# PimLb/POMDP_PBVI_Exploration

Hardware: AMD Instinct MI355X
Metric: alpha-vector backups/sec (higher is better)
Workload: dtype f32

## Files before the change

pomdp_pbvi_exploration_amd/csrc/backup_kernels.h:

```cpp
#pragma once
#include "pbvi_common.h"

namespace pbvi {

template <typename T>
struct ModelView {
    int S, S_pad, A, O, R;
    const int32_t* rs;
    const T* rto;
    const T* er;
    const uint8_t* sup;
};

__host__ __device__ __forceinline__ int64_t push_row_index(int o, int a, int b, int A, int B) {
#ifdef PBVI_PUSH_ORDER_OAB
    return ((int64_t)o * A + a) * B + b;
#else
    return ((int64_t)o * B + b) * A + a;
#endif
}

template <typename T>
struct SlabView {
    const T* slabs;
// ... 51 lines not shown
hipError_t launch_dead(const T* bel, int ldb, int B, ModelView<T> mv,
                       const unsigned long long* nzBw ,
                       int k_tiles, uint8_t* dead, int32_t* btl ,
                       int32_t* btc , int* dead_count ,
                       hipStream_t st, const uint8_t* rowflags = nullptr ,
                       const int32_t* perm = nullptr );

template <typename T>
hipError_t launch_push_project(const T* bel, int ldb, int B, ModelView<T> mv, const int32_t* in_ptr,
                               const int32_t* in_src, double gamma, const T* amax, T* bp, int ldp, double* mag,
                               hipStream_t st, uint8_t* nzP = nullptr );
template <typename T>
hipError_t launch_rdot(const T* bel, int ldb, int B, ModelView<T> mv, const int32_t* btl, const int32_t* btc, double* rd,
                       hipStream_t st);

template <typename T>
hipError_t launch_argmax(SlabView<T> sv, int V, int G, int B, const uint8_t* dead, double tol_rel, double tol_abs,
                         const int* chain_steps ,
                         int flag_all, int32_t* best_v, double* best_score, double* err, int32_t* queue, int* qcount,
                         hipStream_t st, double tol_extra = 0.0 ,
                         int split = 0 );

template <typename T>
hipError_t launch_fold_chunk(SlabView<T> sv, int B, int G, int Vc, int V, int v0, int tail_cols, T* dst, int64_t ldd,
                             const int* chain, int* chain_max, hipStream_t st);

struct RefineWork {
    int32_t* items_v = nullptr;
    int32_t* items_slot = nullptr;
    double* scores = nullptr;
    int32_t* slot_entry = nullptr;
    int32_t* slot_n = nullptr;
    int32_t* tiles = nullptr;
    unsigned long long* emax = nullptr;
    int32_t* eidx = nullptr;
    double* ib_val = nullptr;
// ... 15 lines not shown
    int* klistW = nullptr;
    int* kcountW = nullptr;
    const int32_t* in_ptr = nullptr;
    const int32_t* in_src = nullptr;
    const float* gam = nullptr;
    int ldg = 0;
    double l1_rel = 0.0;
};

template <typename T, typename TS>
hipError_t launch_refine(bool proj, SlabView<TS> sv, int V, int G, int max_entries, const int32_t* queue,
                         const int* qcount, const T* bel, int ldb, const T* alpha, int lda, ModelView<T> mv,
                         double gamma, const int32_t* btl, const int32_t* btc ,
                         const uint8_t* nzG ,
                         int32_t* best_v, double* best_score, double* err, int* cand_total ,
                         RefineWork work, hipStream_t st);

template <typename T, typename TS>
hipError_t launch_refine_scan(bool proj, SlabView<TS> sv, int V, int G, int max_entries, const int32_t* queue,
                              const int* qcount, const T* bel, int ldb, const T* alpha, int lda, ModelView<T> mv,
                              double gamma, const int32_t* btl, const int32_t* btc, const uint8_t* nzG, int32_t* best_v,
                              double* best_score, double* err, int* cand_total, RefineWork work, int* counts_host,
                              hipStream_t st);
template <typename T>
hipError_t launch_refine_deferred(bool proj, int V, int G, const T* bel, int ldb, const T* alpha, int lda, ModelView<T> mv,
                                  double gamma, int32_t* best_v, double* best_score, double* err, RefineWork work,
                                  int h_items, int h_slots, hipStream_t st);

template <typename T>
hipError_t launch_belief_tiles(const T* bel, int ldb, int B, int S, int k_tiles, int32_t* btl, int32_t* btc,
                               hipStream_t st);

template <typename T>
hipError_t launch_tail_rows(ModelView<T> mv, T* gam , int64_t row0 , int ldg, hipStream_t st,
                            const int32_t* ctile = nullptr);
template <typename T>
hipError_t launch_action(int B, ModelView<T> mv, SlabView<T> sv, int64_t rd_col0, double tol_rel, const int* chain_steps,
                         const double* best_score, const double* err, double* rdot, double* rdot_err, int32_t* action,
// ... 46 lines not shown
```

pomdp_pbvi_exploration_amd/csrc/backup_kernels.hip:

```cpp
#include "backup_kernels.h"

#include <cstdlib>
#include <limits>

namespace pbvi {

__device__ __forceinline__ double wave_sum(double v) {
#pragma unroll
    for (int off = 32; off > 0; off >>= 1) v += __shfl_xor(v, off, 64);
    return v;
}

__device__ __forceinline__ double block_sum(double v, double* sh) {
    v = wave_sum(v);
    const int lane = threadIdx.x & 63, wid = threadIdx.x >> 6;
    __syncthreads();
    if (lane == 0) sh[wid] = v;
    __syncthreads();
    return ((sh[0] + sh[1]) + sh[2]) + sh[3];
}

struct TileList {
    const int32_t* list;
    int count;
// ... 567 lines not shown
    return hipGetLastError();
}

__device__ __forceinline__ double score_window(double tol_rel, const int* chain_steps, int split) {
    const double u24 = 5.9604644775390625e-08;
    double tr = tol_rel;
    if (chain_steps != nullptr && tol_rel < 0.0)
        tr = 8.0 * u24 * (sqrt((double)chain_steps[0] * 32.0 * (split ? 3.0 : 1.0)) + 1.0);
    if (split) tr = (tr + 3.1 * 1.52587890625e-05) * (1.0 + 4.8828125e-04);
    return tr;
}

template <typename T>
__global__ void k_argmax(SlabView<T> sv, int V, int G, int B, const uint8_t* __restrict__ dead, double tol_rel,
                         double tol_abs, double tol_extra, const int* __restrict__ chain_steps, int flag_all, int32_t* __restrict__ best_v, double* __restrict__ best_score,
                         double* __restrict__ err, int32_t* __restrict__ queue, int* __restrict__ qcount, int split) {
    const int lane = threadIdx.x & 63;
    const int64_t gw = (int64_t)blockIdx.x * 4 + (threadIdx.x >> 6);
    if (gw >= (int64_t)B * G) return;
    const int b = (int)(gw / G), g = (int)(gw % G);
    if (dead != nullptr && dead[gw]) {
        if (lane == 0) {
            best_v[gw] = 0;
            best_score[gw] = 0.0;
            err[gw] = 0.0;
        }
        return;
    }
    T m = -std::numeric_limits<T>::infinity(), m2 = -std::numeric_limits<T>::infinity();
    int idx = 0x7fffffff;
    bool vec4 = false;
// ... 81 lines not shown
        if (oi != 0x7fffffff && idx != 0x7fffffff) n2 = lo > n2 ? lo : n2;
        if (om > m || (om == m && oi < idx)) {
            m = om;
            idx = oi;
        }
        m2 = n2;
    }
    double E = 0.0;
    int push = 0;
    if (queue != nullptr) {
        const double mag = fmax(fabs((double)m), fabs(sv.magnitude(b, g, G, V)));
        const double tr = score_window(tol_rel, chain_steps, split) + (sv.push ? 2.0 * 5.9604644775390625e-08 : 0.0);
        E = (tr + tol_extra) * mag + tol_abs;
        push = (flag_all || (double)m2 >= (double)m - 2.0 * E) ? 1 : 0;
    }
    if (lane == 0) {
        best_v[gw] = idx;
        best_score[gw] = (double)m;
        err[gw] = E;
        if (push) {
            const int slot = atomicAdd(qcount, 1);
            queue[slot] = (int32_t)gw;
        }
    }
}

template <typename T>
hipError_t launch_argmax(SlabView<T> sv, int V, int G, int B, const uint8_t* dead, double tol_rel, double tol_abs,
                         const int* chain_steps, int flag_all, int32_t* best_v, double* best_score, double* err,
                         int32_t* queue, int* qcount, hipStream_t st, double tol_extra, int split) {
    const int64_t rows = (int64_t)B * G;
    if (rows <= 0) return hipSuccess;
    hipLaunchKernelGGL(k_argmax<T>, dim3((unsigned)((rows + 3) / 4)), dim3(256), 0, st, sv, V, G, B, dead, tol_rel,
                       tol_abs, tol_extra, chain_steps, flag_all, best_v, best_score, err, queue, qcount, split);
    return hipGetLastError();
}

template <typename T>
__global__ void k_fold_chunk(SlabView<T> sv, int B, int G, int Vc, int V, int v0, int tail_cols, T* __restrict__ dst,
                             int64_t ldd, const int* __restrict__ chain, int* __restrict__ chain_max) {
    if (chain != nullptr && blockIdx.x == 0 && blockIdx.y == 0 && threadIdx.x == 0) {
        const int c = chain[0];
        if (c > chain_max[0]) chain_max[0] = c;
    }
    const int64_t group_cols = (int64_t)G * Vc, n_cols = group_cols + tail_cols;
    const int64_t j0 = ((int64_t)blockIdx.x * 256 + threadIdx.x) * 4;
    if (j0 >= n_cols) return;
    bool vec4 = false;
    if constexpr (sizeof(T) == 4) vec4 = sv.nchunks != nullptr && (Vc & 3) == 0 && (sv.ldc & 3) == 0 && j0 + 3 < group_cols;
// ... 81 lines not shown
            }
#pragma unroll
            for (int j = 0; j < 4; ++j) acc[j] += w[j] * ((double)brow[s[j]] * (gamma * g[j]));
        } else {
#pragma unroll
            for (int j = 0; j < 4; ++j) {
                const bool in = s[j] < mv.S;
                acc[j] += (in ? w[j] : 0.0) * ((double)brow[s[j]] * (double)arow[in ? s[j] : 0]);
            }
        }
    }
    return wave_sum((acc[0] + acc[1]) + (acc[2] + acc[3]));
}

template <typename T, typename TS, bool PROJ, bool L1 >
__global__ void k_refine(SlabView<TS> sv, int V, int G, const int32_t* __restrict__ queue,
                         const int* __restrict__ qcount,
                         const T* __restrict__ bel, int ldb, const T* __restrict__ alpha, int lda,
                         ModelView<T> mv, double gamma, const int32_t* __restrict__ btl, const int32_t* __restrict__ btc,
                         const uint8_t* __restrict__ nzG ,
                         int32_t* __restrict__ best_v,
                         double* __restrict__ best_score, double* __restrict__ err, int* __restrict__ cand_total,
                         RefineWork work) {
    __shared__ int cand[256];
    __shared__ int wcount[4];
    __shared__ int ltile[REFINE_LIST_CAP];
    __shared__ int lbase, loverflow;
    __shared__ int sh_slot, sh_base;
    __shared__ double red[4];
    __shared__ double wbest[4];
    __shared__ int widx[4];
    if ((int)blockIdx.x >= *qcount) return;
    const int tid = threadIdx.x, lane = tid & 63, wid = tid >> 6;
    const int e = queue[blockIdx.x];
    const int b = e / G, g = e % G;
    const int a = PROJ ? g / mv.O : 0, o = PROJ ? g % mv.O : 0;
    const double m = best_score[e], E = err[e];
    const double thr = m - 2.0 * E;
    const T* brow = bel + (int64_t)b * ldb;
    const int k_tiles = mv.S_pad >> 5;
    const int32_t* src = btl ? btl + (int64_t)b * k_tiles : nullptr;
    const int n_src = btl ? btc[b] : k_tiles;
    const uint8_t* zg = (PROJ && nzG) ? nzG + (int64_t)g * k_tiles : nullptr;
    if (tid == 0) {
        lbase = 0;
        loverflow = 0;
    }
    __syncthreads();
    for (int i0 = 0; i0 < n_src; i0 += 256) {
        const int i = i0 + tid;
        int t = 0, f = 0;
        if (i < n_src) {
            t = src ? src[i] : i;
            f = zg ? (zg[t] != 0) : 1;
        }
        const unsigned long long mask = __ballot(f);
        if (lane == 0) wcount[wid] = __popcll(mask);
        __syncthreads();
        int off = lbase;
        for (int w = 0; w < wid; ++w) off += wcount[w];
        const int tot = wcount[0] + wcount[1] + wcount[2] + wcount[3];
        const bool fits = lbase + tot <= REFINE_LIST_CAP;
        if (f && fits) ltile[off + __popcll(mask & ((1ull << lane) - 1ull))] = t;
        __syncthreads();
        if (tid == 0) {
            if (fits) lbase += tot;
            else loverflow = 1;
        }
        __syncthreads();
        if (loverflow) break;
    }
    const int* L = loverflow ? src : ltile;
    const int n_tiles = loverflow ? n_src : lbase;

    double bestval = -std::numeric_limits<double>::infinity();
    int bestidx = 0x7fffffff;
    int slot = -1;
    if (tid == 0) sh_slot = -1;
    auto score_exact = [&](int ncand) {
        if (ncand <= 2) {
            const TileList tl{L, n_tiles};
            for (int c = 0; c < ncand; ++c) {
                const int vv = cand[c];
                const T* arow = alpha + (int64_t)vv * lda;
                const double part = PROJ ? proj_dot_partial(brow, arow, mv, a, o, gamma, tl)
// ... 11 lines not shown
                if (tot > bestval) {
                    bestval = tot;
                    bestidx = vv;
                }
            }
        }
    };
    bool settled = false;
    if (!loverflow) {
        constexpr int L1_CAP = 32;
        constexpr int FAST_CAP = 8;
        __shared__ int c1[L1_CAP];
        __shared__ double s1[L1_CAP];
        __shared__ double l1red[16];
        __shared__ int n1_sh, n2_sh;
        if (tid == 0) n1_sh = 0;
        __syncthreads();
        for (int v0 = 0; v0 < V; v0 += 256) {
            const int v = v0 + tid;
            int flag = 0;
            if (v < V) flag = ((double)sv.score(b, g, V, v) >= thr) ? 1 : 0;
            const unsigned long long mask = __ballot(flag);
            if (lane == 0) wcount[wid] = __popcll(mask);
            __syncthreads();
            int base = n1_sh;
            for (int w = 0; w < wid; ++w) base += wcount[w];
            const int pos = base + __popcll(mask & ((1ull << lane) - 1ull));
            if (flag && pos < L1_CAP) c1[pos] = v;
            __syncthreads();
            if (tid == 0) n1_sh += wcount[0] + wcount[1] + wcount[2] + wcount[3];
            __syncthreads();
        }
        const int n1 = n1_sh;
        constexpr bool l1 = L1 && PROJ && sizeof(T) == 4;
        if (n1 > 0 && n1 <= L1_CAP && (l1 || n1 <= FAST_CAP)) {
            if (tid == 0 && cand_total != nullptr) atomicAdd(cand_total, n1);
            const TileList tl{L, n_tiles};
            int n2 = n1;
            if constexpr (l1) {
                {
                    for (int c0 = 0; c0 < n1; c0 += 4) {
                        const float* rows[4];
#pragma unroll
                        for (int j = 0; j < 4; ++j)
                            rows[j] = work.gam + ((int64_t)g * V + c1[c0 + j < n1 ? c0 + j : c0]) * work.ldg;
                        double d[4];
// ... 138 lines not shown
                bv = wbest[w];
                bi = widx[w];
            }
        if (slot >= 0 && slot < work.w_slot_cap) {
        } else if (slot >= 0) {
            work.ib_val[slot] = bv;
            work.ib_idx[slot] = bi;
        } else if (bi != 0x7fffffff) {
            best_v[e] = bi;
            best_score[e] = bv;
            err[e] = 0.0;
        }
    }
}

template <typename T, bool PROJ>
__global__ void k_refine_split(int G, const T* __restrict__ bel, int ldb, const T* __restrict__ alpha, int lda, ModelView<T> mv,
                               double gamma, const int32_t* __restrict__ btl, const int32_t* __restrict__ btc,
                               const uint8_t* __restrict__ nzG, int32_t* __restrict__ best_v, double* __restrict__ best_score,
                               double* __restrict__ err, RefineWork work) {
    __shared__ int wcount[4];
    __shared__ int ltile[REFINE_LIST_CAP];
    __shared__ int lbase, loverflow, last;
    __shared__ double red16[16];
    const int tid = threadIdx.x, lane = tid & 63, wid = tid >> 6, part = blockIdx.y;
    const int n_q = min(work.cnt[2], work.q2_cap);
    const int k_tiles = mv.S_pad >> 5;
    for (int q = blockIdx.x; q < n_q; q += gridDim.x) {
        const int e = work.q2_entry[q], nc_all = work.q2_n[q];
        const int b = e / G, g = e % G;
// ... 197 lines not shown
    if (tid == 0) {
        for (int w = 1; w < 4; ++w)
            if (wv[w] > m || (wv[w] == m && wi[w] < idx)) {
                m = wv[w];
                idx = wi[w];
            }
        if (idx != 0x7fffffff) {
            const int e = work.slot_entry[sl];
            best_v[e] = idx;
            best_score[e] = m;
            err[e] = 0.0;
        }
    }
}

template <typename T, typename TS>
hipError_t launch_refine_scan(bool proj, SlabView<TS> sv, int V, int G, int max_entries, const int32_t* queue,
                              const int* qcount, const T* bel, int ldb, const T* alpha, int lda, ModelView<T> mv,
                              double gamma, const int32_t* btl, const int32_t* btc, const uint8_t* nzG, int32_t* best_v,
                              double* best_score, double* err, int* cand_total, RefineWork work, int* counts_host,
                              hipStream_t st) {
    if (max_entries <= 0) return hipSuccess;
    hipError_t e;
    if (work.items_v != nullptr) {
        if ((e = hipMemsetAsync(work.cnt, 0, work.zero_bytes, st)) != hipSuccess) return e;
    }
    if (proj)
    {
        if (work.gam != nullptr && sizeof(T) == 4) {
            hipLaunchKernelGGL((k_refine<T, TS, true, true>), dim3(max_entries), dim3(256), 0, st, sv, V, G, queue, qcount, bel, ldb,
                               alpha, lda, mv, gamma, btl, btc, nzG, best_v, best_score, err, cand_total, work);
            if (work.q2_entry != nullptr)
                hipLaunchKernelGGL((k_refine_split<T, true>), dim3(work.q2_cap < 256 ? work.q2_cap : 256, REFINE_SPLIT), dim3(256), 0,
                                   st, G, bel, ldb, alpha, lda, mv, gamma, btl, btc, nzG, best_v, best_score, err, work);
        } else
            hipLaunchKernelGGL((k_refine<T, TS, true, false>), dim3(max_entries), dim3(256), 0, st, sv, V, G, queue, qcount, bel, ldb,
                               alpha, lda, mv, gamma, btl, btc, nzG, best_v, best_score, err, cand_total, work);
    }
    else
        hipLaunchKernelGGL((k_refine<T, TS, false, false>), dim3(max_entries), dim3(256), 0, st, sv, V, G, queue, qcount, bel,
                           ldb, alpha, lda, mv, gamma, btl, btc, nzG, best_v, best_score, err, cand_total, work);
    if ((e = hipGetLastError()) != hipSuccess) return e;
    if (work.items_v != nullptr && counts_host != nullptr)
        if ((e = hipMemcpyAsync(counts_host, work.cnt, 2 * sizeof(int), hipMemcpyDeviceToHost, st)) != hipSuccess) return e;
    return hipSuccess;
}

template <typename T>
hipError_t launch_refine_deferred(bool proj, int V, int G, const T* bel, int ldb, const T* alpha, int lda, ModelView<T> mv,
                                  double gamma, int32_t* best_v, double* best_score, double* err, RefineWork work,
                                  int h_items, int h_slots, hipStream_t st) {
    hipError_t e;
    if (work.items_v == nullptr) return hipSuccess;
    const int n_items = h_items < work.item_cap ? h_items : work.item_cap;
    const int n_slots = h_slots < work.slot_cap ? h_slots : work.slot_cap;
    const int n_w = n_slots < work.w_slot_cap ? n_slots : work.w_slot_cap;
// ... 30 lines not shown
        else
            hipLaunchKernelGGL((k_refine_items<T, false>), dim3(blocks), dim3(256), 0, st, G, bel, ldb, alpha, lda, mv,
                               gamma, work);
        if ((e = hipGetLastError()) != hipSuccess) return e;
        hipLaunchKernelGGL(k_refine_first, dim3(1024), dim3(256), 0, st, work);
        if ((e = hipGetLastError()) != hipSuccess) return e;
    }
    if (n_slots > n_w) hipLaunchKernelGGL(k_refine_merge, dim3(64), dim3(256), 0, st, work, best_v, best_score, err);
    return hipGetLastError();
}

template <typename T, typename TS>
hipError_t launch_refine(bool proj, SlabView<TS> sv, int V, int G, int max_entries, const int32_t* queue,
                         const int* qcount, const T* bel, int ldb, const T* alpha, int lda, ModelView<T> mv,
                         double gamma, const int32_t* btl, const int32_t* btc, const uint8_t* nzG, int32_t* best_v,
                         double* best_score, double* err, int* cand_total, RefineWork work, hipStream_t st) {
    if (max_entries <= 0) return hipSuccess;
    int h_cnt[2] = {0, 0};
    hipError_t e = launch_refine_scan<T, TS>(proj, sv, V, G, max_entries, queue, qcount, bel, ldb, alpha, lda, mv, gamma, btl,
                                             btc, nzG, best_v, best_score, err, cand_total, work, h_cnt, st);
    if (e != hipSuccess || work.items_v == nullptr) return e;
    if ((e = hipStreamSynchronize(st)) != hipSuccess) return e;
    return launch_refine_deferred<T>(proj, V, G, bel, ldb, alpha, lda, mv, gamma, best_v, best_score, err, work, h_cnt[0],
                                     h_cnt[1], st);
}

template <typename T>
__global__ void k_tail_rows(ModelView<T> mv, T* __restrict__ gam, int64_t row0, int ldg, const int32_t* __restrict__ ctile) {
    const int s = blockIdx.x * 256 + threadIdx.x;
    const int j = blockIdx.y;
    if (s >= mv.S_pad) return;
    const T e = mv.er[(int64_t)(j % mv.A) * mv.S_pad + s];
    const int64_t row = row0 + j;
    const int64_t at = ctile != nullptr ? (int64_t)ctile[row >> 8] * 256 + (row & 255) : row;
    gam[at * ldg + s] = (j < mv.A) ? e : (e < T(0) ? -e : e);
// ... 646 lines not shown
    if (e != hipSuccess) return e;
    hipLaunchKernelGGL(k_walk_norm<T>, dim3(blocks), dim3(256), 0, st, unnorm, partial, blocks, mv.S, mv.S_pad, out64,
                       out_store);
    return hipGetLastError();
}

#define PBVI_INST(T)                                                                                                   \
    template hipError_t launch_support<T>(ModelView<T>, uint8_t*, hipStream_t);                                        \
    template hipError_t launch_project<T>(const T*, int, int, ModelView<T>, T, T*, int, const uint8_t*, int,           \
                                          hipStream_t, const uint8_t*, const int*, int, const int32_t*, const int32_t*); \
    template hipError_t launch_tail_rows<T>(ModelView<T>, T*, int64_t, int, hipStream_t, const int32_t*);               \
    template hipError_t launch_dead<T>(const T*, int, int, ModelView<T>, const unsigned long long*, int, uint8_t*, int32_t*, \
                                       int32_t*, int*, hipStream_t, const uint8_t*, const int32_t*);                                                   \
    template hipError_t launch_belief_tiles<T>(const T*, int, int, int, int, int32_t*, int32_t*, hipStream_t);         \
    template hipError_t launch_argmax<T>(SlabView<T>, int, int, int, const uint8_t*, double, double, const int*, int,  \
                                         int32_t*, double*, double*, int32_t*, int*, hipStream_t, double, int);        \
    template hipError_t launch_fold_chunk<T>(SlabView<T>, int, int, int, int, int, int, T*, int64_t, const int*, int*,   \
                                             hipStream_t);                                                             \
    template hipError_t launch_refine<T, T>(bool, SlabView<T>, int, int, int, const int32_t*, const int*, const T*, int, \
                                         const T*, int, ModelView<T>, double, const int32_t*, const int32_t*,          \
                                         const uint8_t*, int32_t*, double*, double*, int*, RefineWork, hipStream_t);   \
    template hipError_t launch_action<T>(int, ModelView<T>, SlabView<T>, int64_t, double, const int*, const double*,   \
                                         const double*, double*, double*, int32_t*, int32_t*, int*, hipStream_t, double, uint8_t*, \
                                         int);                                                                          \
    template hipError_t launch_refine_action<T>(const T*, int, int, const T*, int, ModelView<T>, double,               \
                                                const int32_t*, const int32_t*, const int32_t*, const int*,            \
                                                const double*, const double*, const int32_t*, const double*,           \
                                                const double*, double*, int32_t*, hipStream_t, const uint8_t*);                        \
    template hipError_t launch_assemble<T>(const T*, int, ModelView<T>, double, const int32_t*, const int32_t*,        \
                                           const int32_t*, const int*, int, T*, int, hipStream_t);                     \
    template hipError_t launch_expand_rows<T>(const T*, const int32_t*, T*, int, int, hipStream_t);                    \
    template hipError_t launch_keep<T>(const T*, int, const T*, int, int, int, const double*, const int32_t*,          \
                                       const int32_t*, uint8_t*, hipStream_t);                                         \
    template hipError_t launch_belief_update<T>(const T*, int, int, ModelView<T>, const int32_t*, const int32_t*,      \
                                                const int32_t*, const int32_t*, const int32_t*, double*, double*, T*,  \
                                                int, hipStream_t);                                                     \
// ... 2 lines not shown
    template hipError_t launch_rdot<T>(const T*, int, int, ModelView<T>, const int32_t*, const int32_t*, double*,      \
                                       hipStream_t);                                                                   \
    template hipError_t launch_walk_step<T>(const double*, ModelView<T>, const double*, const int32_t*, const int32_t*, \
                                            int, int, double*, double*, double*, T*, hipStream_t);                     \
    template hipError_t launch_walk_fused<T>(const double*, const double*, const double*, double*, T*, ModelView<T>,      \
                                             const double*, const int32_t*, const int32_t*, int, int, double*, double*,   \
                                             hipStream_t);                                                               \
    template hipError_t launch_walk_finish<T>(const double*, const double*, ModelView<T>, double*, T*, hipStream_t);     \
    template hipError_t launch_dominated<T>(const T*, int, int, int, int*, hipStream_t);
PBVI_INST(float)
PBVI_INST(double)
#define PBVI_INST_REFINE(T, TS)                                                                                        \
    template hipError_t launch_refine_scan<T, TS>(bool, SlabView<TS>, int, int, int, const int32_t*, const int*, const T*, \
                                                  int, const T*, int, ModelView<T>, double, const int32_t*, const int32_t*, \
                                                  const uint8_t*, int32_t*, double*, double*, int*, RefineWork, int*,   \
                                                  hipStream_t);
PBVI_INST_REFINE(float, float)
PBVI_INST_REFINE(double, double)
PBVI_INST_REFINE(double, float)
template hipError_t launch_refine_deferred<float>(bool, int, int, const float*, int, const float*, int, ModelView<float>, double,
                                                  int32_t*, double*, double*, RefineWork, int, int, hipStream_t);
template hipError_t launch_refine_deferred<double>(bool, int, int, const double*, int, const double*, int, ModelView<double>,
                                                   double, int32_t*, double*, double*, RefineWork, int, int, hipStream_t);
template hipError_t launch_refine<double, float>(bool, SlabView<float>, int, int, int, const int32_t*, const int*, const double*,
                                                 int, const double*, int, ModelView<double>, double, const int32_t*,
                                                 const int32_t*, const uint8_t*, int32_t*, double*, double*, int*, RefineWork,
                                                 hipStream_t);

}
```

pomdp_pbvi_exploration_amd/csrc/engine.hip:

```cpp
#include <algorithm>
#include <cmath>
#include <cstdio>
#include <cstdlib>
#include <cstring>
#include <condition_variable>
#include <mutex>
#include <new>
#include <string>
#include <thread>
#include <unistd.h>
#include <vector>

#include "backup_kernels.h"
#include "split_bf16.h"

namespace pbvi {

static thread_local std::string g_err;
static int g_poison = -1;
static bool poison_enabled() {
    if (g_poison < 0) g_poison = getenv("PBVI_POISON") != nullptr ? 1 : 0;
    return g_poison == 1;
}
void set_error(const std::string& msg) { g_err = msg; }
// ... 586 lines not shown
        const int64_t n = (V + lo - 1) / lo;
        Vc = round_up((V + n - 1) / n, 4);
    }
    out->chunk_rows = Vc;
    out->n_chunks = (V + Vc - 1) / Vc;
    out->bytes = bytes_of(Vc);
    return out->bytes <= budget ? PBVI_OK : PBVI_ENOMEM;
}

struct ScoreIO {
    int32_t* best_v;
    double* best_score;
    double* err;
    int32_t* queue;
    int* qcount;
    const uint8_t* dead;
    const double* prd;
    hipEvent_t join;
    hipStream_t side;
    hipEvent_t* ev;
    bool stats;
    double tol_extra;
    bool allow_split;
};
template <typename TS>
struct ScoreStage {
    SlabView<TS> sv;
    GemmPlan plan;
    double tol_rel;
    const int* chain;
// ... 74 lines not shown
    double tie_rel_user_ = -1.0;

    DevBuf rs_, rto_, er_, sup_;
    DevBuf alpha_, alpha_buf_, alpha_small_;
    std::vector<int32_t> prim_ids_;
    int64_t prim_off_ = 0;
    bool prim_valid_ = false, alpha_on_primary_ = false;
    uint64_t prim_layout_ver_ = 0;
    uint64_t screen_layout_seen_ = 0;
    int64_t screen_off_seen_ = 0;
    int64_t V_ = 0;
    DevBuf bel_;
    int64_t B_ = 0, B_pad_ = 0;
    DevBuf belsp_;
    uint64_t belsp_ver_ = 0;
    DevBuf gam_, slabs_, best_v_, best_score_, err_, dead_, queue_, counters_, rdot_, action_, aqueue_, out_, keep_;
    DevBuf bv2_, bs2_, err2_, queue2_, prune_cnt_;
    int tiling_mode_ = 0;
    int64_t tiling_rows_ = 0;
    DevBuf scores_, chain_max_;
    std::vector<hipEvent_t> tile_ev_;
    int tile_ev_chunks_ = 0;
    DevBuf stage_, keys_, perm_, action_res_, best_res_;
    DevBuf rep_, uniq_, inv_, slot_, out_full_;
    DevBuf store_[2], ids_;
    int64_t store_rows_[2] = {0, 0};
    DevBuf in_ptr_, in_src_, bu_act_, bu_obs_, bu_row_, bu_unnorm_, bu_mass_, bu_out_, walk64_, rto64_;
    std::vector<int32_t> h_rs_;
    DevBuf btl_, btc_, val_exact_;
    DevBuf bp_, nzP_, pmag_, prd_;
    bool btl_valid_ = false;
// ... 77 lines not shown
    bool owns_streams_ = true;
    EngineT<float>* screen_ = nullptr;
    std::vector<int32_t> h_reach_ref_;
    std::vector<double> h_rto_ref_, h_er_ref_;
    uint64_t alpha_ver_ = 1, bel_ver_ = 1;
    uint64_t screen_alpha_seen_ = 0, screen_bel_seen_ = 0;

    ~EngineT() override {
        (void)hipSetDevice(device_);
        if (screen_) {
            (void)hipStreamSynchronize(stream_);
            delete screen_;
            screen_ = nullptr;
        }
        DevBuf* all[] = {&rs_, &rto_, &er_, &sup_, &alpha_buf_, &alpha_small_, &bel_, &belsp_, &gam_, &slabs_, &best_v_, &best_score_, &err_,
                         &dead_, &queue_, &counters_, &rdot_, &action_, &aqueue_, &out_, &keep_, &bv2_, &bs2_,
                         &err2_, &queue2_, &prune_cnt_, &nzB_, &nzA_, &klist_, &kcount_, &nchunks_, &need_, &skws_, &stage_, &keys_, &perm_,
                         &action_res_, &best_res_, &rep_, &uniq_, &inv_, &slot_, &out_full_, &btl_, &btc_, &val_exact_, &store_[0], &store_[1], &ids_, &in_ptr_, &in_src_, &bu_act_, &bu_obs_,
                         &bu_unnorm_, &bu_mass_, &bu_out_, &bu_row_, &walk64_, &rto64_, &bp_, &nzP_, &pmag_, &prd_, &keys_tmp_, &keys_act_, &keys_best_, &keys_rows_, &rf_v_, &rf_slot_, &rf_sc_, &rf_entry_, &rf_n_, &rf_tiles_,
                         &snz_, &sbtl_, &sbtc_, &vmax_bk_, &rf_ibv_, &rf_ibi_, &rf_cnt_, &rf_W_, &rf_Cx_, &rf_nzW_, &rf_klW_, &rf_kcW_,
                         &dense_, &nzD_, &nzAlpha_, &prod_, &klistD_, &kcountD_, &nchunksD_, &mat_, &vlist_, &irr_, &rowflags_, &nzBw_, &scr_flag_, &ctile_, &acand_, &rf_q2_, &rf_q2p_, &rf_q2d_, &e_bv_, &e_bs_, &e_err_, &e_rdot_, &e_act_, &e_ares_, &e_bres_, &e_rep_, &e_uniq_, &e_inv_, &e_slotd_, &e_cnt_, &e_out_, &e_slot_, &scores_, &chain_max_};
        static const bool dbg = getenv("PBVI_DEBUG") != nullptr;
        auto chk = [&](hipError_t e, const char* what) {
            if (e != hipSuccess && dbg) fprintf(stderr, "[pbvi] engine teardown: %s: %s\n", what, hipGetErrorString(e));
        };
        for (auto& e : walk_ev_)
            if (e) chk(hipEventDestroy(e), "hipEventDestroy(walk)");
        for (DevBuf* b : all) b->release();
        for (auto& e : tile_ev_)
            if (e) chk(hipEventDestroy(e), "hipEventDestroy(tile)");
        if (host_stage_) chk(hipHostFree(host_stage_), "hipHostFree(stage)");
// ... 700 lines not shown
        int rc = keys_tmp_.ensure((size_t)n * sizeof(uint64_t), &bytes_);
        if (rc) return rc;
        hipLaunchKernelGGL(k_row_hash<double>, dim3((unsigned)n), dim3(256), 0, stream_, walk64_.as<double>() + S_, S_, S_,
                           keys_tmp_.as<unsigned long long>());
        HIPCHK(hipGetLastError());
        if ((rc = out_begin())) return rc;
        if ((rc = out_add(out_keys, keys_tmp_.p, (size_t)n * sizeof(uint64_t)))) return rc;
        return out_finish();
    }

    int after_oom() override {
        HIPCHK(hipSetDevice(device_));
        (void)hipStreamSynchronize(stream_);
        if (stream2_) (void)hipStreamSynchronize(stream2_);
        if (stream3_) (void)hipStreamSynchronize(stream3_);
        DevBuf* drop[] = {&alpha_buf_, &alpha_small_, &bel_, &belsp_, &gam_, &slabs_, &best_v_, &best_score_, &err_, &dead_, &queue_, &rdot_,
                          &action_, &aqueue_, &out_, &keep_, &bv2_, &bs2_, &err2_, &queue2_, &prune_cnt_, &nzA_, &klist_, &kcount_,
                          &nchunks_, &need_, &skws_, &stage_, &keys_, &perm_, &action_res_, &best_res_, &rep_, &uniq_, &inv_, &slot_,
                          &out_full_, &btl_, &btc_, &val_exact_, &store_[0], &store_[1], &ids_, &bu_act_, &bu_obs_, &bu_unnorm_,
                          &bu_mass_, &bu_out_, &bu_row_, &walk64_, &bp_, &nzP_, &pmag_, &prd_, &keys_tmp_, &keys_act_, &keys_best_,
                          &keys_rows_, &rf_v_, &rf_slot_, &rf_sc_, &rf_entry_, &rf_n_, &rf_tiles_, &snz_, &sbtl_, &sbtc_, &vmax_bk_,
                          &rf_ibv_, &rf_ibi_, &rf_cnt_, &rf_W_, &rf_Cx_, &rf_nzW_, &rf_klW_, &rf_kcW_, &nzAlpha_, &prod_, &klistD_,
                          &kcountD_, &nchunksD_, &mat_, &vlist_, &rowflags_, &ctile_, &acand_, &rf_q2_, &rf_q2p_, &rf_q2d_, &e_bv_, &e_bs_, &e_err_, &e_rdot_, &e_act_, &e_ares_, &e_bres_, &e_rep_, &e_uniq_, &e_inv_, &e_slotd_, &e_out_, &e_slot_, &scores_};
        for (DevBuf* b : drop) {
            bytes_ -= (int64_t)b->cap;
            b->release();
        }
        alpha_ = DevBuf{};
        V_ = 0;
        B_ = B_pad_ = 0;
        prim_valid_ = alpha_on_primary_ = false;
// ... 1130 lines not shown
        int split = want_split;
        if ((rc = score_gemm(gam_.as<T>(), N, nzB_.as<uint8_t>(), AO, (int)V_, &sv, nullptr, 0, nullptr, io.side, fused, &split)))
            return rc;
        out->split = split;
        out->fused = fused != nullptr;
    }
    HIPCHK(hipEventRecord(io.ev[2], stream_));
    HIPCHK(hipStreamWaitEvent(stream_, io.join, 0));
    out->plan = plan_;
    const int k_chunk = kF32 ? plan_.chunk_len * GEMM_BK : S_pad_;
    out->tol_rel = tie_window(k_chunk);
    out->chain = chain_steps();
    out->rd_col0 = (int64_t)AO * Vt;
    out->f64_pairs = f64_pairs_;
    HIPCHK(launch_argmax<T>(sv, (int)V_, AO, (int)B_, io.dead, out->tol_rel, 0.0, out->chain, 0, io.best_v, io.best_score,
                            io.err, io.queue, io.qcount, stream_, io.tol_extra, out->split));
    HIPCHK(hipEventRecord(io.ev[3], stream_));
    out->sv = sv;
    return PBVI_OK;
}

template <typename T>
int EngineT<T>::ensure_exact(DevBuf& b, size_t bytes) {
    if (bytes > b.cap && b.p != nullptr) {
        HIPCHK(hipStreamSynchronize(stream_));
        bytes_ -= (int64_t)b.cap;
        b.release();
    }
    return b.ensure(bytes, &bytes_);
}

// ... 72 lines not shown
    full.slabs = scores_.as<T>();
    full.slab_stride = 0;
    full.ldc = (int)ldd;
    full.nchunks = nullptr;
    full.tiles_m = 0;
    full.fixed = 1;
    out->plan = plan_;
    out->tol_rel = on_device ? -1.0 : tol;
    out->chain = on_device ? chain_max_.as<int>() : nullptr;
    out->rd_col0 = (int64_t)AO * Vt;
    out->extra_row0 = -1;
    out->f64_pairs = f64_pairs_;
    out->fused = false;
    out->chunks = (int)n_chunks;
    HIPCHK(launch_argmax<T>(full, (int)V_, AO, (int)B_, io.dead, out->tol_rel, 0.0, out->chain, 0, io.best_v, io.best_score,
                            io.err, io.queue, io.qcount, stream_, io.tol_extra, out->split));
    HIPCHK(hipEventRecord(io.ev[3], stream_));
    out->sv = full;
    return PBVI_OK;
}

template <typename T>
int EngineT<T>::ensure_screen() {
    if constexpr (kF32) {
        return PBVI_OK;
    } else {
        if (screen_) return PBVI_OK;
        if (h_rto_ref_.empty()) FAIL(PBVI_ERUNTIME, "screen: host tables were not kept");
        std::vector<float> rto32(h_rto_ref_.begin(), h_rto_ref_.end()), er32(h_er_ref_.begin(), h_er_ref_.end());
        auto* e = new (std::nothrow) EngineT<float>();
        if (!e) FAIL(PBVI_ENOMEM, "screen: host allocation failed");
// ... 106 lines not shown
    constexpr bool windows = sizeof(TS) == 4;
    constexpr bool screened = sizeof(TS) != sizeof(T);
    int rc;
    const int AO = A_ * O_;
    const int64_t Vt = V_ + 1;
    const int64_t N = (int64_t)AO * Vt + 2 * A_;
    const int64_t pairs = B_ * AO;
    if (N > 0x7fffffff || pairs > 0x7fffffff) FAIL(PBVI_EUNSUPPORTED, "backup_run: A*O*(V+1) or B*A*O exceeds int32");
    const ModelView<T> mv = view();
    const bool use_push = scorer.choose_push(N);
    last_formulation_ = use_push ? 2 : 1;
    if ((rc = best_v_.ensure((size_t)pairs * sizeof(int32_t), &bytes_))) return rc;
    if ((rc = best_score_.ensure((size_t)pairs * sizeof(double), &bytes_))) return rc;
    if ((rc = err_.ensure((size_t)pairs * sizeof(double), &bytes_))) return rc;
    if ((rc = queue_.ensure((size_t)pairs * sizeof(int32_t), &bytes_))) return rc;
    if ((rc = dead_.ensure((size_t)pairs, &bytes_))) return rc;
    if ((rc = rdot_.ensure((size_t)B_ * A_ * 2 * sizeof(double), &bytes_))) return rc;
    if ((rc = action_.ensure((size_t)B_ * sizeof(int32_t), &bytes_))) return rc;
    if ((rc = aqueue_.ensure((size_t)B_ * sizeof(int32_t), &bytes_))) return rc;
    if ((rc = acand_.ensure((size_t)B_ * A_, &bytes_))) return rc;
    if ((rc = out_.ensure((size_t)B_ * S_ * sizeof(T), &bytes_))) return rc;
    if ((rc = keep_.ensure((size_t)B_, &bytes_))) return rc;
    int* qcount = counters_.as<int>();
    int* aqcount = counters_.as<int>() + 1;
    if (windows && (rc = stage_reserve(256))) return rc;
    HIPCHK(hipMemsetAsync(counters_.p, 0, 8 * sizeof(int), stream_));

    HIPCHK(hipEventRecord(ev_[0], stream_));
    static const bool no_side = getenv("PBVI_NO_SIDE_STREAM") != nullptr;
    hipStream_t side = no_side ? stream_ : stream2_;
// ... 27 lines not shown
                              windows ? btc_.as<int32_t>() : nullptr, prd_.as<double>(), side));
    }
    const bool early_wanted = windows && early_rows_ != nullptr && !(flags & PBVI_BELIEF_DOMINANCE) && early_cap_ >= B_ && !no_side;
    if (early_wanted) {
        if ((rc = e_cnt_.ensure(4 * sizeof(int), &bytes_))) return rc;
        HIPCHK(hipMemsetAsync(e_cnt_.p, 0, 4 * sizeof(int), side));
    }
    HIPCHK(hipEventRecord(ev_join_, side));

    ScoreIO io;
    io.best_v = best_v_.as<int32_t>();
    io.best_score = best_score_.as<double>();
    io.err = err_.as<double>();
    io.queue = windows ? queue_.as<int32_t>() : nullptr;
    io.qcount = qcount;
    io.dead = windows ? dead_.as<uint8_t>() : nullptr;
    io.prd = use_push ? prd_.as<double>() : nullptr;
    io.join = ev_join_;
    io.side = lists;
    io.ev = ev_;
    io.stats = st != nullptr;
    io.tol_extra = screened ? 4.0 * 5.9604644775390625e-08 : 0.0;
    io.allow_split = !screened;
    if (windows && !use_push && scorer.tiling_mode_ != 0) {
        RefineWork reserve;
        if ((rc = refine_work(pairs, V_, &reserve))) return rc;
    }
    ScoreStage<TS> sc;
    if ((rc = scorer.stage_scores(gamma, use_push, io, &sc))) return rc;
    const SlabView<TS>& sv = sc.sv;
// ... 87 lines not shown
            if (!no_l1 && !use_push && !sc.fused && sc.chunks <= 1 && mode_ == PBVI_SPARSE) {
                work.gam = (const float*)gam_.p;
                work.ldg = S_pad_;
                work.l1_rel = (double)(R_ + 4) * 5.9604644775390625e-08;
            }
        }
        rf_counts_ = pinned_flag();
        if (!rf_counts_) FAIL(PBVI_ENOMEM, "backup_run: pinned flag");
        rf_counts_ += 24;
        rf_counts_[0] = rf_counts_[1] = 0;
        static const bool no_spec = getenv("PBVI_NO_SPECULATION") != nullptr;
        speculate = !no_spec && last_deferred_nothing_ && work.items_v != nullptr && !(flags & PBVI_BELIEF_DOMINANCE);
        HIPCHK((launch_refine_scan<T, TS>(true, sv, (int)V_, AO, (int)pairs, queue_.as<int32_t>(), qcount, bel_.as<T>(), S_pad_,
                                          alpha_.as<T>(), S_pad_, mv, gamma, btl_.as<int32_t>(), btc_.as<int32_t>(),
                                          nzB_.as<uint8_t>(), best_v_.as<int32_t>(), best_score_.as<double>(), err_.as<double>(),
                                          counters_.as<int>() + 4, work, rf_counts_, stream_)));
        if (!speculate && work.items_v != nullptr) {
            HIPCHK(hipStreamSynchronize(stream_));
            last_deferred_nothing_ = rf_counts_[0] == 0 && rf_counts_[1] == 0;
            HIPCHK(launch_refine_deferred<T>(true, (int)V_, AO, bel_.as<T>(), S_pad_, alpha_.as<T>(), S_pad_, mv, gamma,
                                             best_v_.as<int32_t>(), best_score_.as<double>(), err_.as<double>(), work,
                                             rf_counts_[0], rf_counts_[1], stream_));
        }
    }
    if (early_used_ && early_dma_pending_) {
        HIPCHK(hipEventSynchronize(ev_early_[0]));
        const int np = h_flag_[8];
        if (np > 0)
            HIPCHK(hipMemcpyAsync(early_rows_, e_out_.p, (size_t)np * S_ * sizeof(T), hipMemcpyDeviceToHost, stream2_));
        HIPCHK(hipEventRecord(ev_early_[1], stream2_));
        early_dma_pending_ = false;
// ... 699 lines not shown
```

Measured before the change: 654,800.

## Precompute refine candidate lists in argmax and make refine grid persistent

The argmax kernel now records, for each queued pair, up to a small fixed number of near-best candidate vectors, and the refine kernel reuses that list instead of rescanning all V scores. The refine kernel also becomes a persistent grid capped at resident occupancy that loops over queue entries, and it builds the tile list with a single-wave ballot compaction instead of block-wide atomics. The aim is to cut redundant score scans and block launch overhead in refine. The cost is extra work and a rescan in argmax for pushed rows, plus a new candidate buffer.

```diff
diff --git a/pomdp_pbvi_exploration_amd/csrc/backup_kernels.h b/pomdp_pbvi_exploration_amd/csrc/backup_kernels.h
--- a/pomdp_pbvi_exploration_amd/csrc/backup_kernels.h
+++ b/pomdp_pbvi_exploration_amd/csrc/backup_kernels.h
@@ -89,12 +89,15 @@
 hipError_t launch_rdot(const T* bel, int ldb, int B, ModelView<T> mv, const int32_t* btl, const int32_t* btc, double* rd,
                        hipStream_t st);
 
+constexpr int REFINE_QCAND = 8;
+bool refine_legacy();
 template <typename T>
 hipError_t launch_argmax(SlabView<T> sv, int V, int G, int B, const uint8_t* dead, double tol_rel, double tol_abs,
                          const int* chain_steps ,
                          int flag_all, int32_t* best_v, double* best_score, double* err, int32_t* queue, int* qcount,
                          hipStream_t st, double tol_extra = 0.0 ,
-                         int split = 0 );
+                         int split = 0 ,
+                         int32_t* qcand = nullptr );
 
 template <typename T>
 hipError_t launch_fold_chunk(SlabView<T> sv, int B, int G, int Vc, int V, int v0, int tail_cols, T* dst, int64_t ldd,
@@ -140,14 +143,15 @@
                          double gamma, const int32_t* btl, const int32_t* btc ,
                          const uint8_t* nzG ,
                          int32_t* best_v, double* best_score, double* err, int* cand_total ,
-                         RefineWork work, hipStream_t st);
+                         RefineWork work, hipStream_t st,
+                         const int32_t* qcand = nullptr );
 
 template <typename T, typename TS>
 hipError_t launch_refine_scan(bool proj, SlabView<TS> sv, int V, int G, int max_entries, const int32_t* queue,
                               const int* qcount, const T* bel, int ldb, const T* alpha, int lda, ModelView<T> mv,
                               double gamma, const int32_t* btl, const int32_t* btc, const uint8_t* nzG, int32_t* best_v,
                               double* best_score, double* err, int* cand_total, RefineWork work, int* counts_host,
-                              hipStream_t st);
+                              hipStream_t st, const int32_t* qcand = nullptr);
 template <typename T>
 hipError_t launch_refine_deferred(bool proj, int V, int G, const T* bel, int ldb, const T* alpha, int lda, ModelView<T> mv,
                                   double gamma, int32_t* best_v, double* best_score, double* err, RefineWork work,
diff --git a/pomdp_pbvi_exploration_amd/csrc/backup_kernels.hip b/pomdp_pbvi_exploration_amd/csrc/backup_kernels.hip
--- a/pomdp_pbvi_exploration_amd/csrc/backup_kernels.hip
+++ b/pomdp_pbvi_exploration_amd/csrc/backup_kernels.hip
@@ -2,6 +2,7 @@
 
 #include <cstdlib>
 #include <limits>
+#include <mutex>
 
 namespace pbvi {
 
@@ -605,7 +606,8 @@
 template <typename T>
 __global__ void k_argmax(SlabView<T> sv, int V, int G, int B, const uint8_t* __restrict__ dead, double tol_rel,
                          double tol_abs, double tol_extra, const int* __restrict__ chain_steps, int flag_all, int32_t* __restrict__ best_v, double* __restrict__ best_score,
-                         double* __restrict__ err, int32_t* __restrict__ queue, int* __restrict__ qcount, int split) {
+                         double* __restrict__ err, int32_t* __restrict__ queue, int* __restrict__ qcount, int split,
+                         int32_t* __restrict__ qcand ) {
     const int lane = threadIdx.x & 63;
     const int64_t gw = (int64_t)blockIdx.x * 4 + (threadIdx.x >> 6);
     if (gw >= (int64_t)B * G) return;
@@ -717,25 +719,51 @@
         E = (tr + tol_extra) * mag + tol_abs;
         push = (flag_all || (double)m2 >= (double)m - 2.0 * E) ? 1 : 0;
     }
+    int slot = 0;
     if (lane == 0) {
         best_v[gw] = idx;
         best_score[gw] = (double)m;
         err[gw] = E;
         if (push) {
-            const int slot = atomicAdd(qcount, 1);
+            slot = atomicAdd(qcount, 1);
             queue[slot] = (int32_t)gw;
         }
+    }
+    if (qcand != nullptr && push) {
+        slot = __shfl(slot, 0, 64);
+        int32_t* mine = qcand + (int64_t)slot * (1 + REFINE_QCAND);
+        const double thr = (double)m - 2.0 * E;
+        int n = 0;
+        for (int v0 = 0; v0 < V; v0 += 256) {
+            T sc4[4];
+#pragma unroll
+            for (int j = 0; j < 4; ++j) {
+                const int v = v0 + 64 * j + lane;
+                sc4[j] = v < V ? sv.score(b, g, V, v) : T(0);
+            }
+#pragma unroll
+            for (int j = 0; j < 4; ++j) {
+                const int v = v0 + 64 * j + lane;
+                const int flag = (v < V && (double)sc4[j] >= thr) ? 1 : 0;
+                const unsigned long long mask = __ballot(flag);
+                const int pos = n + __popcll(mask & ((1ull << lane) - 1ull));
+                if (flag && pos < REFINE_QCAND) mine[1 + pos] = v;
+                n += __popcll(mask);
+            }
+        }
+        if (lane == 0) mine[0] = n;
     }
 }
 
 template <typename T>
 hipError_t launch_argmax(SlabView<T> sv, int V, int G, int B, const uint8_t* dead, double tol_rel, double tol_abs,
                          const int* chain_steps, int flag_all, int32_t* best_v, double* best_score, double* err,
-                         int32_t* queue, int* qcount, hipStream_t st, double tol_extra, int split) {
+                         int32_t* queue, int* qcount, hipStream_t st, double tol_extra, int split, int32_t* qcand) {
     const int64_t rows = (int64_t)B * G;
     if (rows <= 0) return hipSuccess;
+    if (queue == nullptr || refine_legacy()) qcand = nullptr;
     hipLaunchKernelGGL(k_argmax<T>, dim3((unsigned)((rows + 3) / 4)), dim3(256), 0, st, sv, V, G, B, dead, tol_rel,
-                       tol_abs, tol_extra, chain_steps, flag_all, best_v, best_score, err, queue, qcount, split);
+                       tol_abs, tol_extra, chain_steps, flag_all, best_v, best_score, err, queue, qcount, split, qcand);
     return hipGetLastError();
 }
 
@@ -847,14 +875,13 @@
 }
 
 template <typename T, typename TS, bool PROJ, bool L1 >
-__global__ void k_refine(SlabView<TS> sv, int V, int G, const int32_t* __restrict__ queue,
-                         const int* __restrict__ qcount,
-                         const T* __restrict__ bel, int ldb, const T* __restrict__ alpha, int lda,
-                         ModelView<T> mv, double gamma, const int32_t* __restrict__ btl, const int32_t* __restrict__ btc,
-                         const uint8_t* __restrict__ nzG ,
-                         int32_t* __restrict__ best_v,
-                         double* __restrict__ best_score, double* __restrict__ err, int* __restrict__ cand_total,
-                         RefineWork work) {
+__device__ __forceinline__ void refine_entry(const SlabView<TS>& sv, int V, int G, const int e, const int32_t* __restrict__ qc,
+                                             const bool wave_list,
+                                             const T* __restrict__ bel, int ldb, const T* __restrict__ alpha, int lda,
+                                             const ModelView<T>& mv, double gamma, const int32_t* __restrict__ btl,
+                                             const int32_t* __restrict__ btc, const uint8_t* __restrict__ nzG,
+                                             int32_t* __restrict__ best_v, double* __restrict__ best_score,
+                                             double* __restrict__ err, int* __restrict__ cand_total, const RefineWork& work) {
     __shared__ int cand[256];
     __shared__ int wcount[4];
     __shared__ int ltile[REFINE_LIST_CAP];
@@ -863,9 +890,9 @@
     __shared__ double red[4];
     __shared__ double wbest[4];
     __shared__ int widx[4];
-    if ((int)blockIdx.x >= *qcount) return;
-    const int tid = threadIdx.x, lane = tid & 63, wid = tid >> 6;
-    const int e = queue[blockIdx.x];
+    int tid_ = threadIdx.x;
+    asm volatile("" : "+v"(tid_));
+    const int tid = tid_, lane = tid & 63, wid = tid >> 6;
     const int b = e / G, g = e % G;
     const int a = PROJ ? g / mv.O : 0, o = PROJ ? g % mv.O : 0;
     const double m = best_score[e], E = err[e];
@@ -875,6 +902,36 @@
     const int32_t* src = btl ? btl + (int64_t)b * k_tiles : nullptr;
     const int n_src = btl ? btc[b] : k_tiles;
     const uint8_t* zg = (PROJ && nzG) ? nzG + (int64_t)g * k_tiles : nullptr;
+    if (wave_list) {
+        if (wid == 0) {
+            int base = 0;
+            for (int i0 = 0; i0 < n_src; i0 += 256) {
+                int t[4], f[4];
+#pragma unroll
+                for (int j = 0; j < 4; ++j) {
+                    const int i = i0 + 64 * j + lane;
+                    t[j] = (i < n_src && src) ? src[i] : i;
+                }
+#pragma unroll
+                for (int j = 0; j < 4; ++j) {
+                    const int i = i0 + 64 * j + lane;
+                    f[j] = i < n_src ? (zg ? (zg[t[j]] != 0) : 1) : 0;
+                }
+#pragma unroll
+                for (int j = 0; j < 4; ++j) {
+                    const unsigned long long mask = __ballot(f[j]);
+                    const int pos = base + __popcll(mask & ((1ull << lane) - 1ull));
+                    if (f[j] && pos < REFINE_LIST_CAP) ltile[pos] = t[j];
+                    base += __popcll(mask);
+                }
+            }
+            if (lane == 0) {
+                lbase = base;
+                loverflow = base > REFINE_LIST_CAP ? 1 : 0;
+            }
+        }
+        __syncthreads();
+    } else {
     if (tid == 0) {
         lbase = 0;
         loverflow = 0;
@@ -902,6 +959,7 @@
         }
         __syncthreads();
         if (loverflow) break;
+    }
     }
     const int* L = loverflow ? src : ltile;
     const int n_tiles = loverflow ? n_src : lbase;
@@ -943,6 +1001,13 @@
         __shared__ double s1[L1_CAP];
         __shared__ double l1red[16];
         __shared__ int n1_sh, n2_sh;
+        static_assert(REFINE_QCAND <= FAST_CAP && REFINE_QCAND <= L1_CAP, "k_argmax's candidate lists feed the fast paths");
+        const int nq = qc != nullptr ? qc[0] : REFINE_QCAND + 1;
+        if (nq <= REFINE_QCAND) {
+            if (tid < nq) c1[tid] = qc[1 + tid];
+            if (tid == 0) n1_sh = nq;
+            __syncthreads();
+        } else {
         if (tid == 0) n1_sh = 0;
         __syncthreads();
         for (int v0 = 0; v0 < V; v0 += 256) {
@@ -959,6 +1024,7 @@
             __syncthreads();
             if (tid == 0) n1_sh += wcount[0] + wcount[1] + wcount[2] + wcount[3];
             __syncthreads();
+        }
         }
         const int n1 = n1_sh;
         constexpr bool l1 = L1 && PROJ && sizeof(T) == 4;
@@ -1127,6 +1193,24 @@
     }
 }
 
+template <typename T, typename TS, bool PROJ, bool L1>
+__global__ void __launch_bounds__(256) __attribute__((amdgpu_waves_per_eu(4))) k_refine(SlabView<TS> sv, int V, int G, const int32_t* __restrict__ queue,
+                         const int* __restrict__ qcount, const int32_t* __restrict__ qcand, int wave_list,
+                         const T* __restrict__ bel, int ldb, const T* __restrict__ alpha, int lda,
+                         ModelView<T> mv, double gamma, const int32_t* __restrict__ btl, const int32_t* __restrict__ btc,
+                         const uint8_t* __restrict__ nzG ,
+                         int32_t* __restrict__ best_v,
+                         double* __restrict__ best_score, double* __restrict__ err, int* __restrict__ cand_total,
+                         RefineWork work) {
+    const int n_q = *qcount;
+    for (int qi = blockIdx.x; qi < n_q; qi += gridDim.x) {
+        if (qi != (int)blockIdx.x) __syncthreads();
+        refine_entry<T, TS, PROJ, L1>(sv, V, G, queue[qi], qcand ? qcand + (int64_t)qi * (1 + REFINE_QCAND) : nullptr,
+                                      wave_list != 0, bel, ldb, alpha, lda, mv, gamma, btl, btc, nzG, best_v, best_score, err,
+                                      cand_total, work);
+    }
+}
+
 template <typename T, bool PROJ>
 __global__ void k_refine_split(int G, const T* __restrict__ bel, int ldb, const T* __restrict__ alpha, int lda, ModelView<T> mv,
                                double gamma, const int32_t* __restrict__ btl, const int32_t* __restrict__ btc,
@@ -1354,32 +1438,69 @@
     }
 }
 
+bool refine_legacy() {
+    static const bool on = getenv("PBVI_REFINE_LEGACY") != nullptr;
+    return on;
+}
+
+static hipError_t refine_resident_blocks(const void* kernel, int* out) {
+    struct Known { const void* kernel; int dev, blocks; };
+    static Known known[16];
+    static int n_known = 0;
+    static std::mutex mu;
+    int dev = 0;
+    hipError_t e;
+    if ((e = hipGetDevice(&dev)) != hipSuccess) return e;
+    std::lock_guard<std::mutex> lock(mu);
+    for (int i = 0; i < n_known; ++i)
+        if (known[i].kernel == kernel && known[i].dev == dev) {
+            *out = known[i].blocks;
+            return hipSuccess;
+        }
+    int per_cu = 0, cus = 0;
+    if ((e = hipOccupancyMaxActiveBlocksPerMultiprocessor(&per_cu, kernel, 256, 0)) != hipSuccess) return e;
+    if ((e = hipDeviceGetAttribute(&cus, hipDeviceAttributeMultiprocessorCount, dev)) != hipSuccess) return e;
+    const int blocks = (per_cu > 0 ? per_cu : 1) * (cus > 0 ? cus : 1);
+    if (n_known < 16) known[n_known++] = Known{kernel, dev, blocks};
+    *out = blocks;
+    return hipSuccess;
+}
+
 template <typename T, typename TS>
 hipError_t launch_refine_scan(bool proj, SlabView<TS> sv, int V, int G, int max_entries, const int32_t* queue,
                               const int* qcount, const T* bel, int ldb, const T* alpha, int lda, ModelView<T> mv,
                               double gamma, const int32_t* btl, const int32_t* btc, const uint8_t* nzG, int32_t* best_v,
                               double* best_score, double* err, int* cand_total, RefineWork work, int* counts_host,
-                              hipStream_t st) {
+                              hipStream_t st, const int32_t* qcand) {
     if (max_entries <= 0) return hipSuccess;
     hipError_t e;
     if (work.items_v != nullptr) {
         if ((e = hipMemsetAsync(work.cnt, 0, work.zero_bytes, st)) != hipSuccess) return e;
     }
+    const bool legacy = refine_legacy();
+    if (legacy) qcand = nullptr;
+    const int wave_list = legacy ? 0 : 1;
+    auto launch = [&](auto kernel) -> hipError_t {
+        int grid = max_entries;
+        if (!legacy) {
+            int resident = 0;
+            if ((e = refine_resident_blocks(reinterpret_cast<const void*>(kernel), &resident)) != hipSuccess) return e;
+            if (resident < grid) grid = resident;
+        }
+        hipLaunchKernelGGL(kernel, dim3(grid), dim3(256), 0, st, sv, V, G, queue, qcount, qcand, wave_list, bel, ldb, alpha, lda, mv,
+                           gamma, btl, btc, nzG, best_v, best_score, err, cand_total, work);
+        return hipGetLastError();
+    };
     if (proj)
     {
         if (work.gam != nullptr && sizeof(T) == 4) {
-            hipLaunchKernelGGL((k_refine<T, TS, true, true>), dim3(max_entries), dim3(256), 0, st, sv, V, G, queue, qcount, bel, ldb,
-                               alpha, lda, mv, gamma, btl, btc, nzG, best_v, best_score, err, cand_total, work);
+            if ((e = launch(k_refine<T, TS, true, true>)) != hipSuccess) return e;
             if (work.q2_entry != nullptr)
                 hipLaunchKernelGGL((k_refine_split<T, true>), dim3(work.q2_cap < 256 ? work.q2_cap : 256, REFINE_SPLIT), dim3(256), 0,
                                    st, G, bel, ldb, alpha, lda, mv, gamma, btl, btc, nzG, best_v, best_score, err, work);
-        } else
-            hipLaunchKernelGGL((k_refine<T, TS, true, false>), dim3(max_entries), dim3(256), 0, st, sv, V, G, queue, qcount, bel, ldb,
-                               alpha, lda, mv, gamma, btl, btc, nzG, best_v, best_score, err, cand_total, work);
-    }
-    else
-        hipLaunchKernelGGL((k_refine<T, TS, false, false>), dim3(max_entries), dim3(256), 0, st, sv, V, G, queue, qcount, bel,
-                           ldb, alpha, lda, mv, gamma, btl, btc, nzG, best_v, best_score, err, cand_total, work);
+        } else if ((e = launch(k_refine<T, TS, true, false>)) != hipSuccess) return e;
+    }
+    else if ((e = launch(k_refine<T, TS, false, false>)) != hipSuccess) return e;
     if ((e = hipGetLastError()) != hipSuccess) return e;
     if (work.items_v != nullptr && counts_host != nullptr)
         if ((e = hipMemcpyAsync(counts_host, work.cnt, 2 * sizeof(int), hipMemcpyDeviceToHost, st)) != hipSuccess) return e;
@@ -1440,11 +1561,12 @@
 hipError_t launch_refine(bool proj, SlabView<TS> sv, int V, int G, int max_entries, const int32_t* queue,
                          const int* qcount, const T* bel, int ldb, const T* alpha, int lda, ModelView<T> mv,
                          double gamma, const int32_t* btl, const int32_t* btc, const uint8_t* nzG, int32_t* best_v,
-                         double* best_score, double* err, int* cand_total, RefineWork work, hipStream_t st) {
+                         double* best_score, double* err, int* cand_total, RefineWork work, hipStream_t st,
+                         const int32_t* qcand) {
     if (max_entries <= 0) return hipSuccess;
     int h_cnt[2] = {0, 0};
     hipError_t e = launch_refine_scan<T, TS>(proj, sv, V, G, max_entries, queue, qcount, bel, ldb, alpha, lda, mv, gamma, btl,
-                                             btc, nzG, best_v, best_score, err, cand_total, work, h_cnt, st);
+                                             btc, nzG, best_v, best_score, err, cand_total, work, h_cnt, st, qcand);
     if (e != hipSuccess || work.items_v == nullptr) return e;
     if ((e = hipStreamSynchronize(st)) != hipSuccess) return e;
     return launch_refine_deferred<T>(proj, V, G, bel, ldb, alpha, lda, mv, gamma, best_v, best_score, err, work, h_cnt[0],
@@ -2121,12 +2243,14 @@
                                        int32_t*, int*, hipStream_t, const uint8_t*, const int32_t*);                                                   \
     template hipError_t launch_belief_tiles<T>(const T*, int, int, int, int, int32_t*, int32_t*, hipStream_t);         \
     template hipError_t launch_argmax<T>(SlabView<T>, int, int, int, const uint8_t*, double, double, const int*, int,  \
-                                         int32_t*, double*, double*, int32_t*, int*, hipStream_t, double, int);        \
+                                         int32_t*, double*, double*, int32_t*, int*, hipStream_t, double, int,          \
+                                         int32_t*);                                                                     \
     template hipError_t launch_fold_chunk<T>(SlabView<T>, int, int, int, int, int, int, T*, int64_t, const int*, int*,   \
                                              hipStream_t);                                                             \
     template hipError_t launch_refine<T, T>(bool, SlabView<T>, int, int, int, const int32_t*, const int*, const T*, int, \
                                          const T*, int, ModelView<T>, double, const int32_t*, const int32_t*,          \
-                                         const uint8_t*, int32_t*, double*, double*, int*, RefineWork, hipStream_t);   \
+                                         const uint8_t*, int32_t*, double*, double*, int*, RefineWork, hipStream_t,    \
+                                         const int32_t*);                                                               \
     template hipError_t launch_action<T>(int, ModelView<T>, SlabView<T>, int64_t, double, const int*, const double*,   \
                                          const double*, double*, double*, int32_t*, int32_t*, int*, hipStream_t, double, uint8_t*, \
                                          int);                                                                          \
@@ -2159,7 +2283,7 @@
     template hipError_t launch_refine_scan<T, TS>(bool, SlabView<TS>, int, int, int, const int32_t*, const int*, const T*, \
                                                   int, const T*, int, ModelView<T>, double, const int32_t*, const int32_t*, \
                                                   const uint8_t*, int32_t*, double*, double*, int*, RefineWork, int*,   \
-                                                  hipStream_t);
+                                                  hipStream_t, const int32_t*);
 PBVI_INST_REFINE(float, float)
 PBVI_INST_REFINE(double, double)
 PBVI_INST_REFINE(double, float)
@@ -2170,6 +2294,6 @@
 template hipError_t launch_refine<double, float>(bool, SlabView<float>, int, int, int, const int32_t*, const int*, const double*,
                                                  int, const double*, int, ModelView<double>, double, const int32_t*,
                                                  const int32_t*, const uint8_t*, int32_t*, double*, double*, int*, RefineWork,
-                                                 hipStream_t);
-
-}
+                                                 hipStream_t, const int32_t*);
+
+}
diff --git a/pomdp_pbvi_exploration_amd/csrc/engine.hip b/pomdp_pbvi_exploration_amd/csrc/engine.hip
--- a/pomdp_pbvi_exploration_amd/csrc/engine.hip
+++ b/pomdp_pbvi_exploration_amd/csrc/engine.hip
@@ -624,6 +624,7 @@
     double* err;
     int32_t* queue;
     int* qcount;
+    int32_t* qcand = nullptr;
     const uint8_t* dead;
     const double* prd;
     hipEvent_t join;
@@ -728,7 +729,7 @@
     int64_t B_ = 0, B_pad_ = 0;
     DevBuf belsp_;
     uint64_t belsp_ver_ = 0;
-    DevBuf gam_, slabs_, best_v_, best_score_, err_, dead_, queue_, counters_, rdot_, action_, aqueue_, out_, keep_;
+    DevBuf gam_, slabs_, best_v_, best_score_, err_, dead_, queue_, qcand_, counters_, rdot_, action_, aqueue_, out_, keep_;
     DevBuf bv2_, bs2_, err2_, queue2_, prune_cnt_;
     int tiling_mode_ = 0;
     int64_t tiling_rows_ = 0;
@@ -836,7 +837,7 @@
             screen_ = nullptr;
         }
         DevBuf* all[] = {&rs_, &rto_, &er_, &sup_, &alpha_buf_, &alpha_small_, &bel_, &belsp_, &gam_, &slabs_, &best_v_, &best_score_, &err_,
-                         &dead_, &queue_, &counters_, &rdot_, &action_, &aqueue_, &out_, &keep_, &bv2_, &bs2_,
+                         &dead_, &queue_, &qcand_, &counters_, &rdot_, &action_, &aqueue_, &out_, &keep_, &bv2_, &bs2_,
                          &err2_, &queue2_, &prune_cnt_, &nzB_, &nzA_, &klist_, &kcount_, &nchunks_, &need_, &skws_, &stage_, &keys_, &perm_,
                          &action_res_, &best_res_, &rep_, &uniq_, &inv_, &slot_, &out_full_, &btl_, &btc_, &val_exact_, &store_[0], &store_[1], &ids_, &in_ptr_, &in_src_, &bu_act_, &bu_obs_,
                          &bu_unnorm_, &bu_mass_, &bu_out_, &bu_row_, &walk64_, &rto64_, &bp_, &nzP_, &pmag_, &prd_, &keys_tmp_, &keys_act_, &keys_best_, &keys_rows_, &rf_v_, &rf_slot_, &rf_sc_, &rf_entry_, &rf_n_, &rf_tiles_,
@@ -1567,7 +1568,7 @@
         (void)hipStreamSynchronize(stream_);
         if (stream2_) (void)hipStreamSynchronize(stream2_);
         if (stream3_) (void)hipStreamSynchronize(stream3_);
-        DevBuf* drop[] = {&alpha_buf_, &alpha_small_, &bel_, &belsp_, &gam_, &slabs_, &best_v_, &best_score_, &err_, &dead_, &queue_, &rdot_,
+        DevBuf* drop[] = {&alpha_buf_, &alpha_small_, &bel_, &belsp_, &gam_, &slabs_, &best_v_, &best_score_, &err_, &dead_, &queue_, &qcand_, &rdot_,
                           &action_, &aqueue_, &out_, &keep_, &bv2_, &bs2_, &err2_, &queue2_, &prune_cnt_, &nzA_, &klist_, &kcount_,
                           &nchunks_, &need_, &skws_, &stage_, &keys_, &perm_, &action_res_, &best_res_, &rep_, &uniq_, &inv_, &slot_,
                           &out_full_, &btl_, &btc_, &val_exact_, &store_[0], &store_[1], &ids_, &bu_act_, &bu_obs_, &bu_unnorm_,
@@ -2728,7 +2729,7 @@
     out->rd_col0 = (int64_t)AO * Vt;
     out->f64_pairs = f64_pairs_;
     HIPCHK(launch_argmax<T>(sv, (int)V_, AO, (int)B_, io.dead, out->tol_rel, 0.0, out->chain, 0, io.best_v, io.best_score,
-                            io.err, io.queue, io.qcount, stream_, io.tol_extra, out->split));
+                            io.err, io.queue, io.qcount, stream_, io.tol_extra, out->split, io.qcand));
     HIPCHK(hipEventRecord(io.ev[3], stream_));
     out->sv = sv;
     return PBVI_OK;
@@ -2831,7 +2832,7 @@
     out->fused = false;
     out->chunks = (int)n_chunks;
     HIPCHK(launch_argmax<T>(full, (int)V_, AO, (int)B_, io.dead, out->tol_rel, 0.0, out->chain, 0, io.best_v, io.best_score,
-                            io.err, io.queue, io.qcount, stream_, io.tol_extra, out->split));
+                            io.err, io.queue, io.qcount, stream_, io.tol_extra, out->split, io.qcand));
     HIPCHK(hipEventRecord(io.ev[3], stream_));
     out->sv = full;
     return PBVI_OK;
@@ -2968,6 +2969,7 @@
     if ((rc = best_score_.ensure((size_t)pairs * sizeof(double), &bytes_))) return rc;
     if ((rc = err_.ensure((size_t)pairs * sizeof(double), &bytes_))) return rc;
     if ((rc = queue_.ensure((size_t)pairs * sizeof(int32_t), &bytes_))) return rc;
+    if (windows && (rc = qcand_.ensure((size_t)pairs * (1 + REFINE_QCAND) * sizeof(int32_t), &bytes_))) return rc;
     if ((rc = dead_.ensure((size_t)pairs, &bytes_))) return rc;
     if ((rc = rdot_.ensure((size_t)B_ * A_ * 2 * sizeof(double), &bytes_))) return rc;
     if ((rc = action_.ensure((size_t)B_ * sizeof(int32_t), &bytes_))) return rc;
@@ -3025,6 +3027,7 @@
     io.err = err_.as<double>();
     io.queue = windows ? queue_.as<int32_t>() : nullptr;
     io.qcount = qcount;
+    io.qcand = windows ? qcand_.as<int32_t>() : nullptr;
     io.dead = windows ? dead_.as<uint8_t>() : nullptr;
     io.prd = use_push ? prd_.as<double>() : nullptr;
     io.join = ev_join_;
@@ -3142,7 +3145,7 @@
         HIPCHK((launch_refine_scan<T, TS>(true, sv, (int)V_, AO, (int)pairs, queue_.as<int32_t>(), qcount, bel_.as<T>(), S_pad_,
                                           alpha_.as<T>(), S_pad_, mv, gamma, btl_.as<int32_t>(), btc_.as<int32_t>(),
                                           nzB_.as<uint8_t>(), best_v_.as<int32_t>(), best_score_.as<double>(), err_.as<double>(),
-                                          counters_.as<int>() + 4, work, rf_counts_, stream_)));
+                                          counters_.as<int>() + 4, work, rf_counts_, stream_, qcand_.as<int32_t>())));
         if (!speculate && work.items_v != nullptr) {
             HIPCHK(hipStreamSynchronize(stream_));
             last_deferred_nothing_ = rf_counts_[0] == 0 && rf_counts_[1] == 0;
```

Result: slower. 622,000 (-5.0%).
